# gabefreedman/fastfp

Hardware: AMD Instinct MI355X
Metric: Fp evals/sec (freqs*draws/s), 67-psr NMFp sweep (higher is better)
Workload: dtype fp64; 1 GPU; model=nmfp, npsr=67, ntoa=5000, basis_size=120, freqs=1000, global_batch=10000, parallelism=dp1 draw-sharded, pool_rotations=4, spectrum_finite=True, pool_draws_redrawn=38

## Files before the change

fastfp_amd/ops/hip/fastfp_kernels.hip:

```cpp

#include <hip/hip_runtime.h>
#include <math.h>

#include <algorithm>

#include "launchers.h"

#define FASTFP_MAXMP 128
#define NB 16

typedef double f64x4 __attribute__((ext_vector_type(4)));
typedef double f64x2 __attribute__((ext_vector_type(2)));

#define MFMA_F64(a, b, c) __builtin_amdgcn_mfma_f64_16x16x4f64((a), (b), (c), 0, 0, 0)

static __device__ __forceinline__ double wave_reduce_sum(double v) {
  for (int off = 32; off > 0; off >>= 1)
    v += __shfl_down(v, off, 64);
  return v;
}

extern "C" __global__ __launch_bounds__(256) void sigdots_kernel(
    const double* __restrict__ toas, const double* __restrict__ ninv,
    const double* __restrict__ nr, const double* __restrict__ freqs,
    int ntoa, int F, double* __restrict__ sNs ,
    double* __restrict__ sNr ) {
  const int f = blockIdx.x;
  if (f >= F) return;
  const double w = 2.0 * M_PI * freqs[f];
  double ss = 0, cc = 0, sc = 0, sr = 0, cr = 0;
  for (int i = threadIdx.x; i < ntoa; i += blockDim.x) {
    double s, c;
    sincos(w * toas[i], &s, &c);
    const double ni = ninv[i];
    const double ri = nr[i];
    ss = fma(s * s, ni, ss);
    cc = fma(c * c, ni, cc);
    sc = fma(s * c, ni, sc);
    sr = fma(s, ri, sr);
    cr = fma(c, ri, cr);
  }
  __shared__ double red[4][5];
  ss = wave_reduce_sum(ss);
  cc = wave_reduce_sum(cc);
  sc = wave_reduce_sum(sc);
  sr = wave_reduce_sum(sr);
  cr = wave_reduce_sum(cr);
  const int lane = threadIdx.x & 63, wv = threadIdx.x >> 6;
  if (lane == 0) {
    red[wv][0] = ss; red[wv][1] = cc; red[wv][2] = sc;
    red[wv][3] = sr; red[wv][4] = cr;
  }
  __syncthreads();
  if (threadIdx.x == 0) {
    double a0 = 0, a1 = 0, a2 = 0, a3 = 0, a4 = 0;
    for (int v = 0; v < 4; ++v) {
      a0 += red[v][0]; a1 += red[v][1]; a2 += red[v][2];
      a3 += red[v][3]; a4 += red[v][4];
    }
    sNs[f] = a0; sNs[F + f] = a1; sNs[2 * F + f] = a2;
    sNr[f] = a3; sNr[F + f] = a4;
  }
}

extern "C" __global__ __launch_bounds__(512) void sbgemm_kernel(
    const double* __restrict__ T ,
    const double* __restrict__ toas, const double* __restrict__ ninv,
    const double* __restrict__ freqs, int ntoa, int m, int mp, int F2,
    double* __restrict__ out, long plane_stride, long ldo) {
  __shared__ double lT[16][FASTFP_MAXMP + 1];
  __shared__ double lS[64][17];

  const int tid = threadIdx.x;
  const int lane = tid & 63;
  const int wv = tid >> 6;
  const int c0 = blockIdx.x * 64;
  const int mbase = blockIdx.z * FASTFP_MAXMP;
  const int mp_loc = min(FASTFP_MAXMP, mp - mbase);
  const int jw = (wv & 3) * 16;
  const int rh = wv >> 2;
  const int rowbase = rh * 64;
  const int nrt_tot = mp_loc >> 4;
  const int rt_lo = min(rh * 4, nrt_tot);
  const int rt_hi = min(rt_lo + 4, nrt_tot);

  const int ks = gridDim.y;
  const int kchunk = (ntoa + ks - 1) / ks;
  const int kbeg = blockIdx.y * kchunk;
  const int kend = min(ntoa, kbeg + kchunk);
  double* outp = out + (long)blockIdx.y * plane_stride;

  f64x4 acc[4];
#pragma unroll
  for (int q = 0; q < 4; ++q) acc[q] = f64x4{0, 0, 0, 0};

  for (int k0 = kbeg; k0 < kend; k0 += 16) {
    for (int idx = tid; idx < 16 * mp_loc; idx += 512) {
      const int k = idx / mp_loc, j = idx % mp_loc;
      const int gk = k0 + k;
      const int gj = mbase + j;
      lT[k][j] = (gk < kend && gj < m) ? T[(long)gk * m + gj] : 0.0;
    }
    for (int idx = tid; idx < 32 * 16; idx += 512) {
      const int p = idx / 16, k = idx % 16;
      const int gk = k0 + k;
      const int ceven = c0 + 2 * p;
      double sv = 0.0, cv = 0.0;
      if (gk < kend && ceven < F2) {
        const double wf = 2.0 * M_PI * freqs[ceven >> 1];
        sincos(wf * toas[gk], &sv, &cv);
        const double ni = ninv[gk];
        sv *= ni; cv *= ni;
      }
      lS[2 * p][k] = sv;
      lS[2 * p + 1][k] = cv;
    }
    __syncthreads();

#pragma unroll
    for (int kk = 0; kk < 4; ++kk) {
      const double b = lS[jw + (lane & 15)][kk * 4 + (lane >> 4)];
#pragma unroll
      for (int q = 0; q < 4; ++q) {
        if (rt_lo + q >= rt_hi) break;
        const double a =
            lT[kk * 4 + (lane >> 4)][rowbase + q * 16 + (lane & 15)];
        acc[q] = MFMA_F64(a, b, acc[q]);
      }
    }
    __syncthreads();
  }

#pragma unroll
  for (int q = 0; q < 4; ++q) {
    if (rt_lo + q >= rt_hi) break;
#pragma unroll
    for (int v = 0; v < 4; ++v) {
      const int row = mbase + rowbase + q * 16 + 4 * v + (lane >> 4);
      const int col = c0 + jw + (lane & 15);
      if (col < F2) outp[(long)row * ldo + col] = acc[q][v];
    }
  }
}

#define A_(i, j) Ash[(i) * ((i) + 3) / 2 + (j)]
#define AS_(i, j) ((j) <= (i) ? A_(i, j) : A_(j, i))


static __device__ __forceinline__ double row_bcast(double w, int t) {
  int lo = __double2loint(w), hi = __double2hiint(w);
  switch (t) {
#define ROW_BCAST_CASE(T)                                                  \
    case T:                                                                \
      lo = __builtin_amdgcn_update_dpp(0, lo, 0x150 + T, 0xF, 0xF, true);  \
      hi = __builtin_amdgcn_update_dpp(0, hi, 0x150 + T, 0xF, 0xF, true);  \
      break;
    ROW_BCAST_CASE(0) ROW_BCAST_CASE(1) ROW_BCAST_CASE(2) ROW_BCAST_CASE(3)
    ROW_BCAST_CASE(4) ROW_BCAST_CASE(5) ROW_BCAST_CASE(6) ROW_BCAST_CASE(7)
    ROW_BCAST_CASE(8) ROW_BCAST_CASE(9) ROW_BCAST_CASE(10) ROW_BCAST_CASE(11)
    ROW_BCAST_CASE(12) ROW_BCAST_CASE(13) ROW_BCAST_CASE(14)
    ROW_BCAST_CASE(15)
#undef ROW_BCAST_CASE
  }
  return __hiloint2double(hi, lo);
}

template <int NBT>
__global__ __launch_bounds__(512, 4) void chol_batch_kernel(
    const double* __restrict__ TNT_all ,
    const double* __restrict__ phiinv_all , int m, int D,
    double* __restrict__ L_all ,
    double* __restrict__ invd_all ) {
  const int pp = blockIdx.y;
  const double* TNT = TNT_all + (long)pp * m * m;
  const double* phiinv = phiinv_all + (long)pp * D * m;
  double* L = L_all + (long)pp * D * (NBT * 16) * (NBT * 16);
  double* invd = invd_all + (long)pp * D * NBT * 256;
  constexpr int mp = NBT * 16;
  __shared__ double Ash[mp * (mp + 3) / 2];
  __shared__ double inv16[2][16][17];

  const int d = blockIdx.x;
  if (d >= D) return;
  const int tid = threadIdx.x;
  const int lane = tid & 63;
  const int wv = tid >> 6;
  constexpr int nb = NBT;

  const int nthr = blockDim.x;
  const int nwv = nthr >> 6;
  for (int idx = tid; idx < mp * mp; idx += nthr) {
    const int i = idx / mp, j = idx % mp;
    if (j > i) continue;
    double v = (i < m && j < m) ? TNT[(long)i * m + j] : 0.0;
    if (i == j) v += (i < m) ? phiinv[(long)d * m + i] : 1.0;
    A_(i, j) = v;
  }
  __syncthreads();

#define CHOL_DIAG(KB, DST)                                                   \
  {                                                                          \
    const int dk0 = (KB)*NB;                                                 \
    const int i = lane & 15;                                                 \
    double row[16];                                                          \
    _Pragma("unroll") for (int c = 0; c < 16; ++c) row[c] =                  \
        AS_(dk0 + i, dk0 + c);                                               \
    _Pragma("unroll") for (int t = 0; t < 16; ++t) {                         \
      const double dv = sqrt(row_bcast(row[t], t));                          \
      double rdv = 1.0 / dv;                                                 \
         \
         \
      asm volatile("" : "+v"(rdv));                                          \
      row[t] = (i == t) ? dv : row[t] * rdv;                                 \
      _Pragma("unroll") for (int j = t + 1; j < 16; ++j)                     \
        row[j] = fma(-row[t], row_bcast(row[t], j), row[j]);                 \
         \
      __builtin_amdgcn_sched_barrier(0);                                     \
    }                                                                        \
    _Pragma("unroll") for (int c = 0; c < 16; ++c) if (c <= i)               \
        A_(dk0 + i, dk0 + c) = row[c];                                       \
    const int c = i;                                                         \
    double x[16];                                                            \
       \
       \
       \
       \
       \
    double dii = 0.0;                                                        \
    _Pragma("unroll") for (int r = 0; r < 16; ++r) if (r == i) dii = row[r]; \
    const double myrcp = 1.0 / dii;                                          \
    _Pragma("unroll") for (int r = 0; r < 16; ++r) {                         \
      const double dr = row_bcast(myrcp, r);                                 \
      double acc2 = 0.0;                                                     \
      _Pragma("unroll") for (int t = 0; t < 16; ++t) {                       \
        const double lrt = row_bcast(row[t], r);                             \
        if (t < r) acc2 = fma(lrt, x[t], acc2);                              \
      }                                                                      \
      x[r] = (r < c) ? 0.0 : (r == c) ? dr : -acc2 * dr;                     \
      __builtin_amdgcn_sched_barrier(0);                                     \
    }                                                                        \
    _Pragma("unroll") for (int r = 0; r < 16; ++r) (DST)[r][c] = x[r];       \
    if (lane < 16)                                                           \
      _Pragma("unroll") for (int r = 0; r < 16; ++r)                         \
          invd[((long)d * nb + (KB)) * 256 + r * 16 + c] = x[r];             \
  }

  if (wv == 0) CHOL_DIAG(0, inv16[0]);
  __syncthreads();

  for (int kb = 0; kb < nb; ++kb) {
    const int k0 = kb * NB;

    for (int rt = kb + 1 + wv; rt < nb; rt += nwv) {
      const int r0 = rt * NB;
      f64x4 pacc = {0, 0, 0, 0};
#pragma unroll
      for (int kk = 0; kk < 4; ++kk) {
        const double a = A_(r0 + (lane & 15), k0 + kk * 4 + (lane >> 4));
        const double b = inv16[kb & 1][lane & 15][kk * 4 + (lane >> 4)];
        pacc = MFMA_F64(a, b, pacc);
      }
#pragma unroll
      for (int v = 0; v < 4; ++v)
        A_(r0 + 4 * v + (lane >> 4), k0 + (lane & 15)) = pacc[v];
    }
    __syncthreads();
    if (kb + 1 >= nb) break;

    const int j1 = (kb + 1) * NB;
    for (int ib = kb + 1 + wv; ib < nb; ib += nwv) {
      const int i0 = ib * NB;
      f64x4 uacc;
#pragma unroll
      for (int v = 0; v < 4; ++v)
        uacc[v] = AS_(i0 + 4 * v + (lane >> 4), j1 + (lane & 15));
#pragma unroll
      for (int kk = 0; kk < 4; ++kk) {
        const double a = -A_(i0 + (lane & 15), k0 + kk * 4 + (lane >> 4));
        const double b = A_(j1 + (lane & 15), k0 + kk * 4 + (lane >> 4));
        uacc = MFMA_F64(a, b, uacc);
      }
#pragma unroll
      for (int v = 0; v < 4; ++v)
        if (i0 + 4 * v + (lane >> 4) >= j1 + (lane & 15))
          A_(i0 + 4 * v + (lane >> 4), j1 + (lane & 15)) = uacc[v];
    }
    __syncthreads();

    if (wv == 0) {
      CHOL_DIAG(kb + 1, inv16[(kb + 1) & 1]);
    } else {
      const int t = nb - kb - 2;
      const int ntile = t * (t + 1) / 2;
      for (int q = wv - 1; q < ntile; q += nwv - 1) {
        int ib = kb + 2, rem = q;
        while (rem > ib - kb - 2) { rem -= (ib - kb - 1); ++ib; }
        const int jb = kb + 2 + rem;
        const int i0 = ib * NB, j0 = jb * NB;
        f64x4 uacc;
#pragma unroll
        for (int v = 0; v < 4; ++v)
          uacc[v] = AS_(i0 + 4 * v + (lane >> 4), j0 + (lane & 15));
#pragma unroll
        for (int kk = 0; kk < 4; ++kk) {
          const double a = -A_(i0 + (lane & 15), k0 + kk * 4 + (lane >> 4));
          const double b = A_(j0 + (lane & 15), k0 + kk * 4 + (lane >> 4));
          uacc = MFMA_F64(a, b, uacc);
        }
#pragma unroll
        for (int v = 0; v < 4; ++v)
          if (i0 + 4 * v + (lane >> 4) >= j0 + (lane & 15))
            A_(i0 + 4 * v + (lane >> 4), j0 + (lane & 15)) = uacc[v];
      }
    }
    __syncthreads();
  }
#undef CHOL_DIAG

  for (int idx = tid; idx < mp * mp; idx += nthr) {
    const int i = idx / mp, j = idx % mp;
    L[((long)d * mp + i) * mp + j] = (j > i) ? 0.0 : A_(i, j);
  }
}

#define FPT_COLS 128
#define FPT_FREQS 63
#define NBMAX (FASTFP_MAXMP / 16)

static __device__ __forceinline__ double fp_close(
    double s11, double s22, double s12, double r1, double r2, double gsign,
    double ss, double cc, double sc, double su, double cu) {
  const double M11 = s11 - gsign * ss;
  const double M22 = s22 - gsign * cc;
  const double M12 = s12 - gsign * sc;
  const double N1 = r1 - gsign * su;
  const double N2 = r2 - gsign * cu;
  const double det = fma(M11, M22, -M12 * M12);
  const double num =
      fma(N1 * N1, M22, fma(-2.0 * N1, N2 * M12, N2 * N2 * M11));
  return 0.5 * num / det;
}

template <int NBT, int DPG, bool PRODS = false>
__global__ __launch_bounds__(512, 4) void trsm_fp_kernel(
    const double* __restrict__ L_all ,
    const double* __restrict__ invd_all ,
    const double* __restrict__ RHS_all ,
    const double* __restrict__ sNs_all ,
    const double* __restrict__ sNr_all , int F, int D,
    double gsign,
    double* __restrict__ fp_all ) {
  constexpr int mp = NBT * 16;
  __shared__ double Lp[2][DPG][16][NBT * 16 + 1];
  __shared__ double Iv[DPG][NBT][16][17];
  __shared__ double Wu[DPG][NBT * 16];

  const int pp = blockIdx.z;
  const double* L = L_all + (long)pp * D * mp * mp;
  const double* invd = invd_all + (long)pp * D * NBT * 256;
  const double* RHS = RHS_all + (long)pp * mp * (2L * F + 1);
  const double* sNs = sNs_all + (long)pp * 3 * F;
  const double* sNr = sNr_all + (long)pp * 2 * F;
  double* fp = fp_all + (long)pp * D * F;
  const int d0 = blockIdx.y * DPG;
  const int f0 = blockIdx.x * FPT_FREQS;
  const int tid = threadIdx.x;
  const int lane = tid & 63;
  const int wv = tid >> 6;
  const long ldr = 2L * F + 1;
  const int jw = wv * 16;
  const int li = lane & 15;
  const int lk = lane >> 4;
  const int ndr = min(DPG, D - d0);

  for (int idx = tid; idx < ndr * NBT * 256; idx += 512) {
    const int e = idx / (NBT * 256);
    const int r = idx % (NBT * 256);
    Iv[e][r >> 8][(r >> 4) & 15][r & 15] =
        invd[((long)(d0 + e) * NBT) * 256 + r];
  }

  const int bc = jw + li;
  f64x4 W[DPG][NBT];
#pragma unroll
  for (int rt = 0; rt < NBT; ++rt) {
#pragma unroll
    for (int v = 0; v < 4; ++v) {
      const long row = rt * 16 + 4 * v + lk;
      double val = 0.0;
      if (bc < 126) {
        const long gc = 2L * f0 + bc;
        if (gc < 2L * F) val = RHS[row * ldr + gc];
      } else if (bc == 126) {
        val = RHS[row * ldr + 2L * F];
      }
#pragma unroll
      for (int e = 0; e < DPG; ++e) W[e][rt][v] = val;
    }
  }
  __syncthreads();

#pragma unroll
  for (int rb = 0; rb < NBT; ++rb) {
    if (rb + 1 < NBT) {
      const int ncols = (rb + 1) * 16;
      for (int idx = tid; idx < ndr * 16 * ncols; idx += 512) {
        const int e = idx / (16 * ncols);
        const int q = idx % (16 * ncols);
        const int r = q / ncols, c = q % ncols;
        Lp[(rb + 1) & 1][e][r][c] =
            L[((long)(d0 + e) * mp + (rb + 1) * 16 + r) * mp + c];
      }
    }
    f64x4 acc[DPG], acc2[DPG];
#pragma unroll
    for (int e = 0; e < DPG; ++e) {
      acc[e] = -W[e][rb];
      acc2[e] = f64x4{0, 0, 0, 0};
    }
#pragma unroll
    for (int cb = 0; cb < rb; ++cb) {
#pragma unroll
      for (int kk = 0; kk < 4; ++kk) {
#pragma unroll
        for (int e = 0; e < DPG; ++e) {
          const double a = Lp[rb & 1][e][li][cb * 16 + kk * 4 + lk];
          if (cb & 1)
            acc2[e] = MFMA_F64(a, W[e][cb][kk], acc2[e]);
          else
            acc[e] = MFMA_F64(a, W[e][cb][kk], acc[e]);
        }
      }
    }
#pragma unroll
    for (int e = 0; e < DPG; ++e) acc[e] += acc2[e];
    f64x4 sol[DPG];
#pragma unroll
    for (int e = 0; e < DPG; ++e) sol[e] = f64x4{0, 0, 0, 0};
#pragma unroll
    for (int kk = 0; kk < 4; ++kk) {
#pragma unroll
      for (int e = 0; e < DPG; ++e) {
        const double a = Iv[e][rb][li][kk * 4 + lk];
        sol[e] = MFMA_F64(a, -acc[e][kk], sol[e]);
      }
    }
#pragma unroll
    for (int e = 0; e < DPG; ++e) W[e][rb] = sol[e];
    __syncthreads();
  }

  if (wv == 7) {
#pragma unroll
    for (int rt = 0; rt < NBT; ++rt)
#pragma unroll
      for (int v = 0; v < 4; ++v)
#pragma unroll
        for (int e = 0; e < DPG; ++e)
          if (li == 14) Wu[e][rt * 16 + 4 * v + lk] = W[e][rt][v];
  }
  __syncthreads();

#pragma unroll
  for (int e = 0; e < DPG; ++e) {
    if (e >= ndr) break;
    double a1 = 0, a2 = 0, a3 = 0;
#pragma unroll
    for (int rt = 0; rt < NBT; ++rt) {
#pragma unroll
      for (int v = 0; v < 4; ++v) {
        const double w = W[e][rt][v];
        const double wp = __shfl_xor(w, 1, 64);
        const double wu = Wu[e][rt * 16 + 4 * v + lk];
        a1 = fma(w, w, a1);
        a2 = fma(w, wu, a2);
        a3 = fma(w, wp, a3);
      }
    }
    a1 += __shfl_down(a1, 32, 64); a1 += __shfl_down(a1, 16, 64);
    a2 += __shfl_down(a2, 32, 64); a2 += __shfl_down(a2, 16, 64);
    a3 += __shfl_down(a3, 32, 64); a3 += __shfl_down(a3, 16, 64);
    const double b1 = __shfl_xor(a1, 1, 64);
    const double b2 = __shfl_xor(a2, 1, 64);
    const int q = (jw + li) >> 1;
    if (lk == 0 && (li & 1) == 0 && q < FPT_FREQS && f0 + q < F) {
      const int f = f0 + q;
      if constexpr (PRODS) {
        double* o = fp_all + (((long)pp * D + (d0 + e)) * 5) * F + f;
        o[0] = sNs[f] - gsign * a1;
        o[F] = sNs[F + f] - gsign * b1;
        o[2L * F] = sNs[2 * F + f] - gsign * a3;
        o[3L * F] = sNr[f] - gsign * a2;
        o[4L * F] = sNr[F + f] - gsign * b2;
      } else {
        fp[(long)(d0 + e) * F + f] +=
            fp_close(sNs[f], sNs[F + f], sNs[2 * F + f], sNr[f], sNr[F + f],
                     gsign, a1, b1, a3, a2, b2);
      }
    }
  }
}

#define DL_BS 18
#define DL_BLK (16 * DL_BS)
#define DL_FREQS 63

static __device__ __forceinline__ double pair_swap(double w) {
  int lo = __double2loint(w), hi = __double2hiint(w);
  lo = __builtin_amdgcn_update_dpp(0, lo, 0xB1, 0xF, 0xF, true);
  hi = __builtin_amdgcn_update_dpp(0, hi, 0xB1, 0xF, 0xF, true);
  return __hiloint2double(hi, lo);
}

template <int NBT, int SKIP, bool PRODS = false>
__global__ __launch_bounds__(512, 4) void trsm_fp_draws_kernel(
    const double* __restrict__ L_all ,
    const double* __restrict__ invd_all ,
    const double* __restrict__ RHS_all ,
    const double* __restrict__ sNs_all ,
    const double* __restrict__ sNr_all , int F, int D, int P,
    int dpb , int nsl ,
    double gsign,
    double* __restrict__ fp_all ) {
  constexpr int mp = NBT * 16;
  constexpr int UC = 126;
  constexpr int NLB = NBT * (NBT - 1) / 2;
  constexpr int BUF = (NLB + NBT) * DL_BLK;
  static_assert(NBT * 128 <= 512, "one prefetch slot per panel");
  __shared__ __attribute__((aligned(16))) double S[2 * BUF + 2 * mp + 5 * 64];

  const int ntile = (F + DL_FREQS - 1) / DL_FREQS;
  const int j = blockIdx.x >> 3;
  const int s = (j / ntile) * 8 + (blockIdx.x & 7);
  if (s >= P * nsl) return;
  const int pp = s / nsl;
  const int dlo = (s % nsl) * dpb;
  const int dhi = min(D, dlo + dpb);
  const int f0 = (j % ntile) * DL_FREQS;

  const double* L = L_all + (long)pp * D * mp * mp;
  const double* invd = invd_all + (long)pp * D * NBT * 256;
  const double* RHS = RHS_all + (long)pp * mp * (2L * F + 1);
  const double* sNs = sNs_all + (long)pp * 3 * F;
  const double* sNr = sNr_all + (long)pp * 2 * F;
  double* fp = fp_all + (long)pp * D * F;
  const int tid = threadIdx.x;
  const int lane = tid & 63;
  const int wv = tid >> 6;
  const long ldr = 2L * F + 1;
  const int jw = wv * 16;
  const int li = lane & 15;
  const int lk = lane >> 4;

  f64x2 pre[NBT];
  auto fetch = [&](int d) {
    const double* Ld = L + (long)d * mp * mp;
    pre[0] = reinterpret_cast<const f64x2*>(
        invd + (long)d * NBT * 256)[min(tid, NBT * 128 - 1)];
#pragma unroll
    for (int rb = 1; rb < NBT; ++rb) {
      const int idx = min(tid, rb * 128 - 1);
      const int r = idx / (rb * 8), c = 2 * (idx % (rb * 8));
      pre[rb] =
          *reinterpret_cast<const f64x2*>(Ld + (rb * 16 + r) * mp + c);
    }
  };
  auto stage = [&](double* buf) {
    if (tid < NBT * 128)
      *reinterpret_cast<f64x2*>(buf + (NLB + (tid >> 7)) * DL_BLK +
                                ((tid >> 3) & 15) * DL_BS + 2 * (tid & 7)) =
          pre[0];
#pragma unroll
    for (int rb = 1; rb < NBT; ++rb) {
      if (tid < rb * 128) {
        const int r = tid / (rb * 8), c = 2 * (tid % (rb * 8));
        *reinterpret_cast<f64x2*>(buf +
                                  (rb * (rb - 1) / 2 + (c >> 4)) * DL_BLK +
                                  r * DL_BS + (c & 15)) = -pre[rb];
      }
    }
  };

  fetch(dlo);

  const int bc = jw + li;
  f64x4 R0[NBT];
#pragma unroll
  for (int rt = 0; rt < NBT; ++rt) {
#pragma unroll
    for (int v = 0; v < 4; ++v) {
      const long row = rt * 16 + 4 * v + lk;
      double val = 0.0;
      if (bc < UC) {
        const long gc = 2L * f0 + bc;
        if (gc < 2L * F) val = RHS[row * ldr + gc];
      } else if (bc == UC) {
        val = RHS[row * ldr + 2L * F];
      }
      R0[rt][v] = val;
    }
  }
  double* Sc = S + 2 * BUF + 2 * mp;
  if (tid < 64) {
    const bool live = tid < DL_FREQS && f0 + tid < F;
    const int fq = live ? f0 + tid : 0;
#pragma unroll
    for (int i = 0; i < 3; ++i)
      Sc[i * 64 + tid] = live ? sNs[i * F + fq] : 0.0;
#pragma unroll
    for (int i = 0; i < 2; ++i)
      Sc[(3 + i) * 64 + tid] = live ? sNr[i * F + fq] : 0.0;
  }
  const int q = bc >> 1;
  const int f = f0 + q;
  const bool closer = lk == 0 && (li & 1) == 0 && q < DL_FREQS && f < F;

  stage(S);
  __syncthreads();

  const int aoff = li * DL_BS + lk;
  for (int d = dlo; d < dhi; ++d) {
    const int b = (d - dlo) & 1;
    const double* Sb = S + b * BUF;
    double* Wu = S + 2 * BUF + b * mp;
    const bool more = d + 1 < dhi;
    if (more) fetch(d + 1);

    f64x4 W[NBT];
    double a1 = 0, a2 = 0, a3 = 0;
#pragma unroll
    for (int rb = 0; rb < NBT; ++rb) {
      f64x4 acc = R0[rb];
      f64x4 acc2 = f64x4{0, 0, 0, 0};
#pragma unroll
      for (int cb = 0; cb < rb; ++cb) {
#pragma unroll
        for (int kk = 0; kk < 4; ++kk) {
          if (cb == 0 && kk < SKIP) continue;
          const double a =
              Sb[(rb * (rb - 1) / 2 + cb) * DL_BLK + kk * 4 + aoff];
          if (cb & 1)
            acc2 = MFMA_F64(a, W[cb][kk], acc2);
          else
            acc = MFMA_F64(a, W[cb][kk], acc);
        }
      }
      acc += acc2;
      f64x4 sol = f64x4{0, 0, 0, 0};
#pragma unroll
      for (int kk = 0; kk < 4; ++kk) {
        if (rb == 0 && kk < SKIP) continue;
        const double a = Sb[(NLB + rb) * DL_BLK + kk * 4 + aoff];
        sol = MFMA_F64(a, acc[kk], sol);
      }
      W[rb] = sol;
#pragma unroll
      for (int v = 0; v < 4; ++v) {
        const double w = sol[v];
        const double wp = pair_swap(w);
        a1 = fma(w, w, a1);
        a3 = fma(w, wp, a3);
      }
      asm volatile("" : "+v"(a1), "+v"(a3));
    }
    if (wv == 7 && li == 14) {
#pragma unroll
      for (int rt = 0; rt < NBT; ++rt)
#pragma unroll
        for (int v = 0; v < 4; ++v) Wu[rt * 16 + 4 * v + lk] = W[rt][v];
    }
    if (more) stage(S + (b ^ 1) * BUF);
    __syncthreads();

#pragma unroll
    for (int rt = 0; rt < NBT; ++rt)
#pragma unroll
      for (int v = 0; v < 4; ++v)
        a2 = fma(W[rt][v], Wu[rt * 16 + 4 * v + lk], a2);
    a1 += __shfl_down(a1, 32, 64); a1 += __shfl_down(a1, 16, 64);
    a2 += __shfl_down(a2, 32, 64); a2 += __shfl_down(a2, 16, 64);
    a3 += __shfl_down(a3, 32, 64); a3 += __shfl_down(a3, 16, 64);
    const double b1 = pair_swap(a1);
    const double b2 = pair_swap(a2);
    if constexpr (PRODS) {
      if (closer) {
        double* o = fp_all + (((long)pp * D + d) * 5) * F + f;
        o[0] = Sc[q] - gsign * a1;
        o[F] = Sc[64 + q] - gsign * b1;
        o[2L * F] = Sc[128 + q] - gsign * a3;
        o[3L * F] = Sc[192 + q] - gsign * a2;
        o[4L * F] = Sc[256 + q] - gsign * b2;
      }
    } else {
      if (closer)
        fp[(long)d * F + f] =
            fp_close(Sc[q], Sc[64 + q], Sc[128 + q], Sc[192 + q], Sc[256 + q],
                     gsign, a1, b1, a3, a2, b2);
    }
  }
}

template <int NBT>
__global__ __launch_bounds__(512, 4) void trsm_fp_rl_kernel(
    const double* __restrict__ L_all ,
    const double* __restrict__ invd_all ,
    const double* __restrict__ RHS_all ,
    const double* __restrict__ sNs_all ,
    const double* __restrict__ sNr_all , int F, int D,
    double gsign, double* __restrict__ fp_all ) {
  constexpr int mp = NBT * 16;
  constexpr int PROWS = NBT > 1 ? (NBT - 1) * 16 : 1;
  __shared__ double Lc[2][PROWS][19];
  __shared__ double Iv[NBT][16][19];
  __shared__ double Wu[NBT * 16];

  const int pp = blockIdx.z;
  const double* L = L_all + (long)pp * D * mp * mp;
  const double* invd = invd_all + (long)pp * D * NBT * 256;
  const double* RHS = RHS_all + (long)pp * mp * (2L * F + 1);
  const double* sNs = sNs_all + (long)pp * 3 * F;
  const double* sNr = sNr_all + (long)pp * 2 * F;
  double* fp = fp_all + (long)pp * D * F;
  const int d0 = blockIdx.y;
  const int f0 = blockIdx.x * FPT_FREQS;
  const int tid = threadIdx.x;
  const int lane = tid & 63;
  const int wv = tid >> 6;
  const long ldr = 2L * F + 1;
  const int jw = wv * 16;
  const int li = lane & 15;
  const int lk = lane >> 4;

  for (int idx = tid; idx < NBT * 256; idx += 512)
    Iv[idx >> 8][(idx >> 4) & 15][idx & 15] =
        invd[(long)d0 * NBT * 256 + idx];

  const int bc = jw + li;
  f64x4 W[NBT];
#pragma unroll
  for (int rt = 0; rt < NBT; ++rt) {
#pragma unroll
    for (int v = 0; v < 4; ++v) {
      const long row = rt * 16 + 4 * v + lk;
      double val = 0.0;
      if (bc < 126) {
        const long gc = 2L * f0 + bc;
        if (gc < 2L * F) val = RHS[row * ldr + gc];
      } else if (bc == 126) {
        val = RHS[row * ldr + 2L * F];
      }
      W[rt][v] = val;
    }
  }

  if (NBT > 1) {
    for (int idx = tid; idx < (NBT - 1) * 16 * 16; idx += 512) {
      const int r = idx >> 4, c = idx & 15;
      Lc[0][r][c] = L[((long)d0 * mp + 16 + r) * mp + c];
    }
  }
  __syncthreads();

#pragma unroll
  for (int cb = 0; cb < NBT; ++cb) {
    f64x4 sol = f64x4{0, 0, 0, 0};
#pragma unroll
    for (int kk = 0; kk < 4; ++kk) {
      const double a = Iv[cb][li][kk * 4 + lk];
      sol = MFMA_F64(a, W[cb][kk], sol);
    }
    W[cb] = sol;
#pragma unroll
    for (int rb = cb + 1; rb < NBT; ++rb) {
#pragma unroll
      for (int kk = 0; kk < 4; ++kk) {
        const double a = -Lc[cb & 1][(rb - cb - 1) * 16 + li][kk * 4 + lk];
        W[rb] = MFMA_F64(a, sol[kk], W[rb]);
      }
    }
    if (cb + 1 < NBT) {
      const int nrows2 = (NBT - 2 - cb) * 16;
      for (int idx = tid; idx < nrows2 * 16; idx += 512) {
        const int r = idx >> 4, c = idx & 15;
        Lc[(cb + 1) & 1][r][c] =
            L[((long)d0 * mp + (cb + 2) * 16 + r) * mp + (cb + 1) * 16 + c];
      }
    }
    __syncthreads();
  }

  if (wv == 7) {
#pragma unroll
    for (int rt = 0; rt < NBT; ++rt)
#pragma unroll
      for (int v = 0; v < 4; ++v)
        if (li == 14) Wu[rt * 16 + 4 * v + lk] = W[rt][v];
  }
  __syncthreads();

  double a1 = 0, a2 = 0, a3 = 0;
#pragma unroll
  for (int rt = 0; rt < NBT; ++rt) {
#pragma unroll
    for (int v = 0; v < 4; ++v) {
      const double w = W[rt][v];
      const double wp = __shfl_xor(w, 1, 64);
      const double wu = Wu[rt * 16 + 4 * v + lk];
      a1 = fma(w, w, a1);
      a2 = fma(w, wu, a2);
      a3 = fma(w, wp, a3);
    }
  }
  a1 += __shfl_down(a1, 32, 64); a1 += __shfl_down(a1, 16, 64);
  a2 += __shfl_down(a2, 32, 64); a2 += __shfl_down(a2, 16, 64);
  a3 += __shfl_down(a3, 32, 64); a3 += __shfl_down(a3, 16, 64);
  const double b1 = __shfl_xor(a1, 1, 64);
  const double b2 = __shfl_xor(a2, 1, 64);
  const int q = (jw + li) >> 1;
  if (lk == 0 && (li & 1) == 0 && q < FPT_FREQS && f0 + q < F) {
    const int f = f0 + q;
    const double M11 = sNs[f] - gsign * a1;
    const double M22 = sNs[F + f] - gsign * b1;
    const double M12 = sNs[2 * F + f] - gsign * a3;
    const double N1 = sNr[f] - gsign * a2;
    const double N2 = sNr[F + f] - gsign * b2;
    const double det = fma(M11, M22, -M12 * M12);
    const double num =
        fma(N1 * N1, M22, fma(-2.0 * N1, N2 * M12, N2 * N2 * M11));
    fp[(long)d0 * F + f] += 0.5 * num / det;
  }
}

extern "C" __global__ __launch_bounds__(512, 4) void diag_inv_kernel(
    const double* __restrict__ L, int mp, long nblk_total,
    double* __restrict__ invd) {
  const long w = (long)blockIdx.x * 8 + (threadIdx.x >> 6);
  if (w >= nblk_total) return;
  const int nbt = mp >> 4;
  const long b = w / nbt;
  const int kb = (int)(w % nbt);
  const int lane = threadIdx.x & 63;
  const int i = lane & 15;
  const double* Lb = L + b * (long)mp * mp + (long)kb * 16 * mp + kb * 16;
  double row[16];
#pragma unroll
  for (int c = 0; c < 16; ++c) row[c] = (c <= i) ? Lb[(long)i * mp + c] : 0.0;
  const int c = i;
  double x[16];
  double dii = 1.0;
#pragma unroll
  for (int r = 0; r < 16; ++r)
    if (r == i) dii = row[r];
  const double myrcp = 1.0 / dii;
#pragma unroll
  for (int r = 0; r < 16; ++r) {
    const double dr = __shfl(myrcp, r, 16);
    double acc = 0.0;
#pragma unroll
    for (int t = 0; t < 16; ++t) {
      const double lrt = __shfl(row[t], r, 16);
      if (t >= c && t < r) acc = fma(lrt, x[t], acc);
    }
    x[r] = (r < c) ? 0.0 : (r == c) ? dr : -acc * dr;
  }
  if (lane < 16)
#pragma unroll
    for (int r = 0; r < 16; ++r)
      invd[(b * nbt + kb) * 256 + r * 16 + c] = x[r];
}


extern "C" __global__ __launch_bounds__(256) void sigdots_block_kernel(
    const double* __restrict__ toas, const double* __restrict__ uvec,
    const double* __restrict__ nr, const double* __restrict__ freqs,
    const double* __restrict__ beta, const long* __restrict__ offsets,
    const long* __restrict__ sizes, int nblk, int ntoa, int F,
    double* __restrict__ sNs, double* __restrict__ sNr) {
  const int f = blockIdx.x;
  if (f >= F) return;
  const double w = 2.0 * M_PI * freqs[f];
  double ss = 0, cc = 0, sc = 0, sr = 0, cr = 0;
  for (int i = threadIdx.x; i < ntoa; i += blockDim.x) {
    double s, c;
    sincos(w * toas[i], &s, &c);
    const double ui = uvec[i];
    const double ri = nr[i];
    ss = fma(s * s, ui, ss);
    cc = fma(c * c, ui, cc);
    sc = fma(s * c, ui, sc);
    sr = fma(s, ri, sr);
    cr = fma(c, ri, cr);
  }
  for (int b = threadIdx.x; b < nblk; b += blockDim.x) {
    const double bb = beta[b];
    if (bb == 0.0) continue;
    const long o = offsets[b];
    const int sz = (int)sizes[b];
    double us = 0.0, uc = 0.0;
    for (int i = 0; i < sz; ++i) {
      double s, c;
      sincos(w * toas[o + i], &s, &c);
      const double ui = uvec[o + i];
      us = fma(s, ui, us);
      uc = fma(c, ui, uc);
    }
    ss = fma(-bb * us, us, ss);
    cc = fma(-bb * uc, uc, cc);
    sc = fma(-bb * us, uc, sc);
  }
  __shared__ double red[4][5];
  ss = wave_reduce_sum(ss);
  cc = wave_reduce_sum(cc);
  sc = wave_reduce_sum(sc);
  sr = wave_reduce_sum(sr);
  cr = wave_reduce_sum(cr);
  const int lane = threadIdx.x & 63, wv = threadIdx.x >> 6;
  if (lane == 0) {
    red[wv][0] = ss; red[wv][1] = cc; red[wv][2] = sc;
    red[wv][3] = sr; red[wv][4] = cr;
  }
  __syncthreads();
  if (threadIdx.x == 0) {
    double a0 = 0, a1 = 0, a2 = 0, a3 = 0, a4 = 0;
    for (int v = 0; v < 4; ++v) {
      a0 += red[v][0]; a1 += red[v][1]; a2 += red[v][2];
      a3 += red[v][3]; a4 += red[v][4];
    }
    sNs[f] = a0; sNs[F + f] = a1; sNs[2 * F + f] = a2;
    sNr[f] = a3; sNr[F + f] = a4;
  }
}

template <bool PRODS>
static int launch_draws(const double* L, const double* invd,
                        const double* RHS, const double* sNs,
                        const double* sNr, int mp, int F, int D, int P,
                        double gsign, double* out, int draws_per_block,
                        int ncu, int lead, hipStream_t stream) {
  if (lead < 0 || lead > 12 || (lead & 3)) return (int)hipErrorInvalidValue;
  const int ntile = (F + DL_FREQS - 1) / DL_FREQS;
  int dpb = draws_per_block, nsl = 0;
  auto plan = [&](auto kern) -> long {
    if (dpb <= 0) {
      int per_cu = 0;
      if (hipOccupancyMaxActiveBlocksPerMultiprocessor(&per_cu, kern, 512,
                                                       0) != hipSuccess ||
          per_cu < 1)
        per_cu = 1;
      const long slots = (long)per_cu * ncu;
      const long units = (long)P * ntile * D;
      dpb = (int)std::min<long>(64, std::max<long>(1, units / (8 * slots)));
      dpb = std::min(dpb, D);
      const int n = (D + dpb - 1) / dpb;
      dpb = (D + n - 1) / n;
    }
    dpb = std::min(dpb, D);
    nsl = (D + dpb - 1) / dpb;
    return ((long)P * nsl + 7) / 8 * 8 * ntile;
  };
  if (mp < 16 || mp > 64 || (mp & 15)) return (int)hipErrorInvalidValue;
  switch ((mp >> 4) * 4 + (lead >> 2)) {
#define DRAWS_CASE(NBT, SKIP) \
    case NBT * 4 + SKIP: { \
      auto kern = trsm_fp_draws_kernel<NBT, SKIP, PRODS>; \
      const long nblk = plan(kern); \
      if (nblk >= (1L << 31)) return (int)hipErrorInvalidValue; \
      hipLaunchKernelGGL(kern, dim3((unsigned)nblk), dim3(512), 0, stream, \
                         L, invd, RHS, sNs, sNr, F, D, P, dpb, nsl, gsign, \
                         out); \
    } break;
#define DRAWS_NBT(NBT) \
    DRAWS_CASE(NBT, 0) DRAWS_CASE(NBT, 1) DRAWS_CASE(NBT, 2) DRAWS_CASE(NBT, 3)
    DRAWS_NBT(1) DRAWS_NBT(2) DRAWS_NBT(3) DRAWS_NBT(4)
#undef DRAWS_NBT
#undef DRAWS_CASE
    default: return (int)hipErrorInvalidValue;
  }
  return (int)hipGetLastError();
}

template <bool PRODS>
static int launch_one_draw(const double* L, const double* invd,
                           const double* RHS, const double* sNs,
                           const double* sNr, int mp, int F, int D, int P,
                           double gsign, double* out, hipStream_t stream) {
  const int ftiles = (F + FPT_FREQS - 1) / FPT_FREQS;
  const dim3 grid(ftiles, D, P), blk(512);
  if (PRODS && mp > FASTFP_MAXMP) return (int)hipErrorInvalidValue;
  switch (mp >> 4) {
#define TRSM_CASE(NBT) \
    case NBT: hipLaunchKernelGGL((trsm_fp_kernel<NBT, 1, PRODS>), grid, blk, \
                  0, stream, L, invd, RHS, sNs, sNr, F, D, gsign, out); break;
    TRSM_CASE(1) TRSM_CASE(2) TRSM_CASE(3) TRSM_CASE(4)
    TRSM_CASE(5) TRSM_CASE(6) TRSM_CASE(7) TRSM_CASE(8)
#undef TRSM_CASE
#define TRSM_BIG_CASE(NBT) \
    case NBT: hipLaunchKernelGGL((trsm_fp_rl_kernel<NBT>), grid, blk, 0, \
                  stream, L, invd, RHS, sNs, sNr, F, D, gsign, out); break;
    TRSM_BIG_CASE(9) TRSM_BIG_CASE(10) TRSM_BIG_CASE(11) TRSM_BIG_CASE(12)
    TRSM_BIG_CASE(13) TRSM_BIG_CASE(14) TRSM_BIG_CASE(15) TRSM_BIG_CASE(16)
#undef TRSM_BIG_CASE
    default: return (int)hipErrorInvalidValue;
  }
  return (int)hipGetLastError();
}

extern "C" {

int launch_sigdots(const double* toas, const double* ninv, const double* nr,
                   const double* freqs, int ntoa, int F, double* sNs,
                   double* sNr, hipStream_t stream) {
  hipLaunchKernelGGL(sigdots_kernel, dim3(F), dim3(256), 0, stream, toas,
                     ninv, nr, freqs, ntoa, F, sNs, sNr);
  return (int)hipGetLastError();
}

int launch_sbgemm(const double* T, const double* toas, const double* ninv,
                  const double* freqs, int ntoa, int m, int mp, int F2,
                  double* out, long plane_stride, long ldo, int ksplit,
                  hipStream_t stream) {
  const int ctiles = (F2 + 63) / 64;
  const int mtiles = (mp + FASTFP_MAXMP - 1) / FASTFP_MAXMP;
  hipLaunchKernelGGL(sbgemm_kernel, dim3(ctiles, ksplit, mtiles), dim3(512),
                     0, stream, T, toas, ninv, freqs, ntoa, m, mp, F2, out,
                     plane_stride, ldo);
  return (int)hipGetLastError();
}

int launch_chol_batch(const double* TNT, const double* phiinv, int m, int mp,
                      int D, int P, double* L, double* invd,
                      hipStream_t stream) {
  const dim3 grid(D, P), blk(mp <= 64 ? 256 : 512);
  switch (mp >> 4) {
#define CHOL_CASE(NBT) \
    case NBT: hipLaunchKernelGGL((chol_batch_kernel<NBT>), grid, blk, \
                  0, stream, TNT, phiinv, m, D, L, invd); break;
    CHOL_CASE(1) CHOL_CASE(2) CHOL_CASE(3) CHOL_CASE(4)
    CHOL_CASE(5) CHOL_CASE(6) CHOL_CASE(7) CHOL_CASE(8)
#undef CHOL_CASE
    default: return (int)hipErrorInvalidValue;
  }
  return (int)hipGetLastError();
}

int launch_trsm(int prods, const double* L, const double* invd,
                const double* RHS, const double* sNs, const double* sNr,
                int mp, int F, int D, int P, double gsign, double* out,
                hipStream_t stream) {
  return prods ? launch_one_draw<true>(L, invd, RHS, sNs, sNr, mp, F, D, P,
                                       gsign, out, stream)
               : launch_one_draw<false>(L, invd, RHS, sNs, sNr, mp, F, D, P,
                                        gsign, out, stream);
}

int trsm_fp_draws_tile_freqs() { return DL_FREQS; }

int launch_trsm_draws(int prods, const double* L, const double* invd,
                      const double* RHS, const double* sNs,
                      const double* sNr, int mp, int F, int D, int P,
                      double gsign, double* out, int draws_per_block,
                      int ncu, int lead, hipStream_t stream) {
  return prods ? launch_draws<true>(L, invd, RHS, sNs, sNr, mp, F, D, P,
                                    gsign, out, draws_per_block, ncu, lead,
                                    stream)
               : launch_draws<false>(L, invd, RHS, sNs, sNr, mp, F, D, P,
                                     gsign, out, draws_per_block, ncu, lead,
                                     stream);
}

int launch_diag_inv(const double* L, int mp, long nblk_total, double* invd,
                    hipStream_t stream) {
  hipLaunchKernelGGL(diag_inv_kernel, dim3((nblk_total + 7) / 8), dim3(512),
                     0, stream, L, mp, nblk_total, invd);
  return (int)hipGetLastError();
}

int launch_sigdots_block(const double* toas, const double* uvec,
                         const double* nr, const double* freqs,
                         const double* beta, const long* offsets,
                         const long* sizes, int nblk, int ntoa, int F,
                         double* sNs, double* sNr, hipStream_t stream) {
  hipLaunchKernelGGL(sigdots_block_kernel, dim3(F), dim3(256), 0, stream,
                     toas, uvec, nr, freqs, beta, offsets, sizes,
                     nblk, ntoa, F, sNs, sNr);
  return (int)hipGetLastError();
}

}
```

Before: 71.69 million evals/s.

## Stream TRSM panels straight into LDS with global_load_lds and negate in MFMA

Replaces the register prefetch of the L and inverse-diagonal panels, and the later LDS store that negates them, with direct global-to-LDS DMA loads. Each thread keeps precomputed source pointers that advance by a fixed stride per draw. The sign flip on the off-diagonal panels moves into the MFMA negate modifier. This is meant to save VGPRs for the prefetch buffers and the ds_write instructions per draw, at the cost of a padded, wave-contiguous LDS layout that also loads duplicate pad elements. It also relies on the compiler waiting on the DMA before the barrier.

```diff
diff --git a/fastfp_amd/ops/hip/fastfp_kernels.hip b/fastfp_amd/ops/hip/fastfp_kernels.hip
--- a/fastfp_amd/ops/hip/fastfp_kernels.hip
+++ b/fastfp_amd/ops/hip/fastfp_kernels.hip
@@ -13,6 +13,7 @@
 typedef double f64x2 __attribute__((ext_vector_type(2)));
 
 #define MFMA_F64(a, b, c) __builtin_amdgcn_mfma_f64_16x16x4f64((a), (b), (c), 0, 0, 0)
+#define MFMA_F64_NEGA(a, b, c) __builtin_amdgcn_mfma_f64_16x16x4f64((a), (b), (c), 0, 0, 1)
 
 static __device__ __forceinline__ double wave_reduce_sum(double v) {
   for (int off = 32; off > 0; off >>= 1)
@@ -526,7 +527,6 @@
   constexpr int UC = 126;
   constexpr int NLB = NBT * (NBT - 1) / 2;
   constexpr int BUF = (NLB + NBT) * DL_BLK;
-  static_assert(NBT * 128 <= 512, "one prefetch slot per panel");
   __shared__ __attribute__((aligned(16))) double S[2 * BUF + 2 * mp + 5 * 64];
 
   const int ntile = (F + DL_FREQS - 1) / DL_FREQS;
@@ -552,36 +552,40 @@
   const int li = lane & 15;
   const int lk = lane >> 4;
 
-  f64x2 pre[NBT];
-  auto fetch = [&](int d) {
-    const double* Ld = L + (long)d * mp * mp;
-    pre[0] = reinterpret_cast<const f64x2*>(
-        invd + (long)d * NBT * 256)[min(tid, NBT * 128 - 1)];
-#pragma unroll
-    for (int rb = 1; rb < NBT; ++rb) {
-      const int idx = min(tid, rb * 128 - 1);
-      const int r = idx / (rb * 8), c = 2 * (idx % (rb * 8));
-      pre[rb] =
-          *reinterpret_cast<const f64x2*>(Ld + (rb * 16 + r) * mp + c);
+  constexpr int NP = (NLB + NBT) * (DL_BLK / 2);
+  constexpr int NPT = (NP + 511) / 512;
+  const double* src[NPT];
+  int inc[NPT];
+#pragma unroll
+  for (int i = 0; i < NPT; ++i) {
+    const int p = min(tid + 512 * i, NP - 1);
+    const int blk = p / (DL_BLK / 2), r = (p % (DL_BLK / 2)) / 9;
+    const int c = 2 * min(p % 9, 7);
+    if (blk < NLB) {
+      const int rb = 1 + (blk >= 1) + (blk >= 3);
+      const int cb = blk - rb * (rb - 1) / 2;
+      src[i] = L + (long)dlo * mp * mp + (rb * 16 + r) * mp + cb * 16 + c;
+      inc[i] = mp * mp;
+    } else {
+      src[i] = invd + (long)dlo * NBT * 256 + (blk - NLB) * 256 + r * 16 + c;
+      inc[i] = NBT * 256;
+    }
+  }
+  const int wvu = __builtin_amdgcn_readfirstlane(wv);
+  auto dma = [&](double* buf) {
+#pragma unroll
+    for (int i = 0; i < NPT; ++i) {
+      if (512 * (i + 1) <= NP || tid + 512 * i < NP)
+        __builtin_amdgcn_global_load_lds(
+            (const __attribute__((address_space(1))) void*)src[i],
+            (__attribute__((address_space(3))) void*)(buf +
+                                                      2 * (512 * i + 64 * wvu)),
+            16, 0, 0);
+      src[i] += inc[i];
     }
   };
-  auto stage = [&](double* buf) {
-    if (tid < NBT * 128)
-      *reinterpret_cast<f64x2*>(buf + (NLB + (tid >> 7)) * DL_BLK +
-                                ((tid >> 3) & 15) * DL_BS + 2 * (tid & 7)) =
-          pre[0];
-#pragma unroll
-    for (int rb = 1; rb < NBT; ++rb) {
-      if (tid < rb * 128) {
-        const int r = tid / (rb * 8), c = 2 * (tid % (rb * 8));
-        *reinterpret_cast<f64x2*>(buf +
-                                  (rb * (rb - 1) / 2 + (c >> 4)) * DL_BLK +
-                                  r * DL_BS + (c & 15)) = -pre[rb];
-      }
-    }
-  };
-
-  fetch(dlo);
+
+  dma(S);
 
   const int bc = jw + li;
   f64x4 R0[NBT];
@@ -615,7 +619,6 @@
   const int f = f0 + q;
   const bool closer = lk == 0 && (li & 1) == 0 && q < DL_FREQS && f < F;
 
-  stage(S);
   __syncthreads();
 
   const int aoff = li * DL_BS + lk;
@@ -623,8 +626,7 @@
     const int b = (d - dlo) & 1;
     const double* Sb = S + b * BUF;
     double* Wu = S + 2 * BUF + b * mp;
-    const bool more = d + 1 < dhi;
-    if (more) fetch(d + 1);
+    if (d + 1 < dhi) dma(S + (b ^ 1) * BUF);
 
     f64x4 W[NBT];
     double a1 = 0, a2 = 0, a3 = 0;
@@ -640,9 +642,9 @@
           const double a =
               Sb[(rb * (rb - 1) / 2 + cb) * DL_BLK + kk * 4 + aoff];
           if (cb & 1)
-            acc2 = MFMA_F64(a, W[cb][kk], acc2);
+            acc2 = MFMA_F64_NEGA(a, W[cb][kk], acc2);
           else
-            acc = MFMA_F64(a, W[cb][kk], acc);
+            acc = MFMA_F64_NEGA(a, W[cb][kk], acc);
         }
       }
       acc += acc2;
@@ -669,7 +671,6 @@
 #pragma unroll
         for (int v = 0; v < 4; ++v) Wu[rt * 16 + 4 * v + lk] = W[rt][v];
     }
-    if (more) stage(S + (b ^ 1) * BUF);
     __syncthreads();
 
 #pragma unroll
```

Result: faster. 73.24 million evals/s (median of 6 runs) (+2.2%).
